# duwt/OrienMask

Measured on AMD Instinct MI355X. Metric: images/sec end-to-end (544^2, bs=32) forward+postprocess, higher is better.
Workload: dtype f32 (fp32 tensors and accumulation; products from hi/lo fp16 pairs of the fp32 operands, three fp16 MFMAs per product group)

## Files before the change

include/orienmask_hip.h:

```cpp
#ifndef ORIENMASK_HIP_H
#define ORIENMASK_HIP_H

#include <stddef.h>
#include <stdint.h>

#ifdef __cplusplus
extern "C" {
#endif

#define OM_VERSION 140

#define OM_OK 0
#define OM_EINVAL (-1)
#define OM_ESTATE (-2)
#define OM_ENOMEM (-3)
#define OM_EHIP (-4)

#define OM_MAX_SCALES 3
#define OM_MAX_ANCHORS 9

typedef struct om_model om_model;
typedef void* om_stream;

typedef struct om_layer_info {
// ... 89 lines not shown
                  void* out, int out_pix_stride, int out_f32, om_stream stream);
int om_conv2d_stem_f16(const float* in, int B, int H, int W, const float* w, const float* scale, const float* shift,
                       int cout, void* out, om_stream stream);
size_t om_conv2d_winograd24_scratch_bytes(int B, int H, int W, int cin);
int om_conv2d_winograd24(const float* in, int B, int H, int W, int cin, int in_pix_stride, const float* u,
                         const float* scale, const float* shift, int cout, int leaky, const float* res,
                         int res_pix_stride, float* out, int out_pix_stride, void* scratch, size_t scratch_bytes,
                         om_stream stream);
int om_conv2d_split(const float* in, int B, int H, int W, int cin, int in_pix_stride, const void* w_split,
                    const float* scale_split, const float* shift, int cout, int ksize, int stride, int leaky, const float* res,
                    int res_pix_stride, float* out, int out_pix_stride, int out_mode, int up, int tile_bm, int tile_bn,
                    int32_t* status_dev, om_stream stream);
int om_conv2d_split_k(const float* in, int B, int H, int W, int cin, int in_pix_stride, const void* w_split,
                      const float* scale_split, const float* shift, int cout, int ksize, int stride, int leaky, const float* res,
                      int res_pix_stride, float* out, int out_pix_stride, int out_mode, int up, int tile_bm, int tile_bn,
                      int max_parts, int32_t* status_dev, om_stream stream);
int om_conv2d_split_gather(int nseg, const float* const* seg_ptr, const int* seg_channels, const int* seg_pix_stride,
                           const int* seg_up, int B, int H, int W, const void* w_split, const float* scale_split, const float* shift,
                           int cout, int leaky, float* out, int out_pix_stride, int32_t* status_dev, om_stream stream);
int om_conv2d_winograd24_split(const float* in, int B, int H, int W, int cin, int in_pix_stride, const void* u_split,
                               const float* scale_split, const float* shift, int cout, int leaky, const float* res,
                               int res_pix_stride, float* out, int out_pix_stride, void* scratch, size_t scratch_bytes,
                               int32_t* status_dev, om_stream stream);
int om_conv2d_wino14_split(const float* in, int B, int H, int W, int cin, int in_pix_stride, const void* u14_split,
                           const float* scale_split, const float* shift, int cout, int leaky, const float* res,
                           int res_pix_stride, float* out, int out_pix_stride, int32_t* status_dev, om_stream stream);
size_t om_conv2d_wino14_wide_scratch_bytes(int B, int H, int W, int cin);
int om_conv2d_wino14_wide(const float* in, int B, int H, int W, int cin, int in_pix_stride, const void* u14_split,
                          const float* scale_split, const float* shift, int cout, int leaky, const float* res,
                          int res_pix_stride, float* out, int out_pix_stride, void* scratch, size_t scratch_bytes,
                          int32_t* status_dev, om_stream stream);
int om_set_wino14_wide(int on);
int om_get_wino14_wide(void);
int om_set_wino14_variant(int variant);
int om_get_wino14_variant(void);
int om_wino14_dual_built(void);
int om_set_stem_fusion(int which, int on);
int om_get_stem_fusion(int which);
int om_set_conv3x3_f16_variant(int mode);
int om_get_conv3x3_f16_variant(void);
int om_conv2d_stem(const float* in, int B, int H, int W, const float* w, const float* scale,
                   const float* shift, int cout, float* out, om_stream stream);
int om_conv2d_stem2_split(const float* in, int B, int H, int W, const float* w1, const float* scale1, const float* shift1,
                          const void* w2_split, const float* scale2_split, const float* shift2, int cout2, int leaky2, float* out,
                          int out_pix_stride, int32_t* status_dev, om_stream stream);
int om_conv2d_stem3_split(const float* in, int B, int H, int W, const float* w1, const float* scale1, const float* shift1,
                          const void* w2_split, const float* scale2_split, const float* shift2, int cout2, int leaky2, float* out,
                          int out_pix_stride, const void* w3_split, const float* scale3_split, const float* shift3, int cout3, int leaky3,
                          float* out3, int out3_pix_stride, int32_t* status_dev, om_stream stream);
int om_conv2d_stem2_f16(const float* in, int B, int H, int W, const float* w1, const float* scale1, const float* shift1,
                        const void* w2_f16, const float* scale2, const float* shift2, int cout2, int leaky2, void* out,
                        int out_pix_stride, om_stream stream);

int om_preprocess(const float* in_nhwc, int N, int h, int w, int resize_h, int resize_w, const float* mean3,
                  const float* std3, int pad_top, int pad_left, int out_h, int out_w, float pad_value, float* out_nchw,
                  om_stream stream);
int om_pad_nchw(const float* in, long long planes, int h, int w, int pad_top, int pad_left, int out_h, int out_w,
                float pad_value, float* out, om_stream stream);

size_t om_postprocess_workspace_bytes(const om_post_cfg* cfg, int B);
int om_postprocess(const om_post_cfg* cfg, const float* bbox32, const float* bbox16, const float* bbox8,
                   const float* oriens, int B, float* out_bbox, int64_t* out_cls, uint8_t* out_mask,
                   int32_t* out_count, int32_t* out_keep, void* workspace, size_t ws_bytes, om_stream stream);
int om_postprocess_detect(const om_post_cfg* cfg, const float* bbox32, const float* bbox16, const float* bbox8, int B,
                          float* out_bbox, int64_t* out_cls, int32_t* out_count, int32_t* out_keep, void* workspace, size_t ws_bytes,
                          om_stream stream);
// ... 119 lines not shown
```

orienmask_amd/csrc/conv_igemm_split.hip:

```cpp
#include <cstdlib>

#include "conv_f16_common.h"

namespace om {

#ifndef OM_SPLIT_WIDE
#define OM_SPLIT_WIDE 1
#endif

#if defined(OM_SPLIT_NO_XCD_PLACEMENT) && !defined(OM_MEASUREMENT_BUILD)
#error "OM_SPLIT_NO_XCD_PLACEMENT is a measurement switch: tools/build_variant.sh only"
#endif
#ifndef OM_SPLIT_TRACE
#define OM_SPLIT_TRACE 0
#endif
#if (OM_SPLIT_TRACE) && !defined(OM_MEASUREMENT_BUILD)
#error "measurement switches (wrong numerics / trace stores) are only for ab/ variants: build them with tools/build_variant.sh, which defines OM_MEASUREMENT_BUILD and never writes orienmask_amd/lib/"
#endif
#if OM_SPLIT_TRACE
static unsigned long long* g_split_trace = nullptr;
extern "C" void om_debug_split_trace(void* buf) { g_split_trace = static_cast<unsigned long long*>(buf); }
#define SPLIT_STAMP(x) asm volatile("s_memtime %0\n\ts_waitcnt lgkmcnt(0)" : "=s"(x)::"memory")
#endif

struct IgemmSParams {
    const _Float16* in;
    const _Float16* w;
    const float* scale;
    const float* shift;
    const float* res;
    float* out;
    int* ticket;
// ... 723 lines not shown
                            for (int g = 0; g < 4; ++g) {
                                const f32x4 v = __builtin_bit_cast(f32x4, __builtin_amdgcn_raw_buffer_load_b128(rs_part, qbase, ((a * TN + b) * 4 + g) * 256 * 16, 16));
#pragma unroll
                                for (int kk = 0; kk < 4; ++kk) acc[a][b][4 * g + kk] += v[kk];
                            }
                }
                asm volatile("s_waitcnt vmcnt(0)" ::: "memory");
            }
        }
#if OM_SPLIT_TRACE
        SPLIT_STAMP(ts2);
#endif

#if OM_SPLIT_TRACE
        SPLIT_STAMP(dts[4]);
#endif
        split_epilogue<BM, BN, WM, WN, FAST>(p, smem, acc, m0, n0, tid, wm, wn, fi, fk, sc, sh);
#if OM_SPLIT_TRACE
        if constexpr (KSPLIT) {
            asm volatile("s_waitcnt vmcnt(0)" ::: "memory");
            SPLIT_STAMP(dts[5]);
            deep_dump();
        }
        SPLIT_STAMP(ts3);
        if (p.trace && blockIdx.x < 16 && n_traced < 16 && tid == 0) {
            unsigned long long* t = p.trace + ((size_t)blockIdx.x * 16 + n_traced) * 8;
            t[0] = ts0; t[1] = ts1; t[2] = ts2; t[3] = ts3; t[4] = twait; t[5] = (unsigned long long)tile;
        }
        ++n_traced;
#endif
    }
}

template <int BM, int BN, int WM, int WN, bool WIDE = false, bool GATHER = false, int NBUF = 3, int WSTAGES = 0>
static int launch_tile_split(IgemmSParams p, int cout_pad, int blocks_per_cu, hipStream_t stream) {
    const int m_tiles = (p.M + BM - 1) / BM;
    p.n_tiles = cout_pad / BN;
    const long long total = (long long)m_tiles * p.n_tiles;
    OM_REQUIRE(total > 0 && total < (1ll << 31), OM_EINVAL, "conv split: %lld tiles out of range", total);
    p.total_tiles = (int)total;
    constexpr bool DEEP = WIDE ? WSTAGES > 2 : NBUF > 3;
    int parts = 1;
    if constexpr (DEEP) {
        if (p.ksplit > 1 && p.partial && total <= SK_SLOTS) {
            parts = p.ksplit;
            if (parts > 512 / (int)total) parts = 512 / (int)total;
            if (parts > p.ksteps / 16) parts = p.ksteps / 16;
            if (parts > 8) parts = 8;
            if (parts < 1) parts = 1;
        }
    }
    p.ksplit = parts;
    p.total_tickets = p.total_tiles * parts;
    p.m_tiles = m_tiles;
    const long long tickets = total * parts;
    long long grid = tickets < 256ll * blocks_per_cu ? tickets : 256ll * blocks_per_cu;
    if constexpr (DEEP) {
        OM_REQUIRE(tickets <= 512, OM_EINVAL, "conv split: %lld units in a deep-ring launch", tickets);
        grid = tickets;
    }
    const bool fast = p.out_mode == 0 && !p.res && p.vec_io && p.cout == cout_pad;
    if constexpr (WIDE) {
        constexpr int WNBUF = DEEP ? WSTAGES : 2;
        if (fast) hipLaunchKernelGGL((conv_igemm_split_wide_kernel<BM, BN, WM, WN, GATHER, true, WNBUF>), dim3((unsigned)grid), dim3(256), 0, stream, p);
        else hipLaunchKernelGGL((conv_igemm_split_wide_kernel<BM, BN, WM, WN, GATHER, false, WNBUF>), dim3((unsigned)grid), dim3(256), 0, stream, p);
    } else {
        if (fast) hipLaunchKernelGGL((conv_igemm_split_kernel<BM, BN, WM, WN, true, NBUF>), dim3((unsigned)grid), dim3(256), 0, stream, p);
        else hipLaunchKernelGGL((conv_igemm_split_kernel<BM, BN, WM, WN, false, NBUF>), dim3((unsigned)grid), dim3(256), 0, stream, p);
    }
    OM_CHECK_HIP(hipGetLastError());
    return OM_OK;
}

void conv_tile_for_split(int M, int cout_pad, int* bm, int* bn) {
    struct Cand { int bm, bn; double eff; };
    const Cand cands[] = {{128, 128, 1.00}, {256, 128, 0.91}, {128, 64, 0.82}, {64, 64, 0.69}, {128, 32, 0.57}};
    double best = 1e300;
    for (const Cand& c : cands) {
        if (cout_pad % c.bn) continue;
        const double cost = (double)((M + c.bm - 1) / c.bm) * (cout_pad / c.bn) * c.bm * c.bn / c.eff;
        if (cost < best) { best = cost; *bm = c.bm; *bn = c.bn; }
    }
#ifndef OM_SPLIT_NO_LATENCY_TILES
    const Cand small[] = {{128, 64, 0}, {64, 64, 0}};
    for (const Cand& c : small) {
        const long long tiles = (long long)((M + *bm - 1) / *bm) * (cout_pad / *bn);
        if (tiles > 128 || cout_pad % c.bn || c.bm * c.bn >= *bm * *bn) continue;
        *bm = c.bm; *bn = c.bn;
    }
#endif
}

int launch_conv_igemm_split(const ConvArgs& a, hipStream_t stream) {
    OM_REQUIRE((a.in || a.nseg > 0) && a.w && a.scale && a.shift && a.out, OM_EINVAL, "conv split: null pointer");
    OM_REQUIRE(a.cin % 16 == 0 && a.cin >= 16, OM_EINVAL, "conv split: cin=%d must be a multiple of 16", a.cin);
    OM_REQUIRE(a.ks == 1 || a.ks == 3, OM_EINVAL, "conv split: ksize=%d not supported", a.ks);
    OM_REQUIRE(a.stride == 1 || a.stride == 2, OM_EINVAL, "conv split: stride=%d not supported", a.stride);
    OM_REQUIRE((a.nseg > 0 || (a.in_pix_stride % 4 == 0 && (reinterpret_cast<uintptr_t>(a.in) & 15) == 0)) &&
                   (reinterpret_cast<uintptr_t>(a.w) & 15) == 0,
               OM_EINVAL, "conv split: input view / weights must be 16-byte aligned");
    OM_REQUIRE(a.cout_pad % 32 == 0 && a.cout <= a.cout_pad, OM_EINVAL, "conv split: cout_pad=%d", a.cout_pad);
    OM_REQUIRE((long long)a.B * a.H * a.W * a.in_pix_stride < (1ll << 40) && (long long)a.B * a.H * a.W < (1ll << 31) &&
// ... 17 lines not shown
    p.total_in_pixels = a.B * a.H * a.W;
    p.w_bytes = a.cout_pad * p.taps * a.cin * 4;
    p.vec_io = (a.out_mode != 2 && a.out_pix_stride % 4 == 0 && (reinterpret_cast<uintptr_t>(a.out) & 15) == 0 &&
                (!a.res || (a.res_pix_stride % 4 == 0 && (reinterpret_cast<uintptr_t>(a.res) & 15) == 0)))
                   ? 1 : 0;
    p.nseg = 0; p.nimg = a.B;
#if OM_SPLIT_TRACE
    p.trace = g_split_trace;
#endif
    for (int g = 0; g < 4; ++g) { p.seg_ptr[g] = p.in; p.seg_stride_h[g] = 0; p.seg_shift[g] = 0; p.seg_end[g] = 0x7FFFFFFF; }
    if (a.nseg > 0) {
        OM_REQUIRE(a.nseg <= 4 && a.ks == 1 && a.stride == 1 && a.cout_pad % 128 == 0, OM_EINVAL,
                   "conv split: a gathered input needs a 1x1 stride-1 layer with cout_pad %% 128 == 0 and at most 4 segments (nseg=%d ks=%d "
                   "stride=%d cout_pad=%d)", a.nseg, a.ks, a.stride, a.cout_pad);
        int end = 0;
        for (int g = 0; g < a.nseg; ++g) {
            const int up = a.seg_up[g];
            int sh = 0;
            while ((1 << sh) < up) ++sh;
            OM_REQUIRE(a.seg_ptr[g] && up >= 1 && (1 << sh) == up && a.H % up == 0 && a.W % up == 0 && a.seg_channels[g] > 0 &&
                           a.seg_channels[g] % 32 == 0 && a.seg_pix_stride[g] % 4 == 0 && a.seg_pix_stride[g] >= a.seg_channels[g] &&
                           (reinterpret_cast<uintptr_t>(a.seg_ptr[g]) & 15) == 0,
                       OM_EINVAL, "conv split: segment %d (channels=%d pix_stride=%d up=%d) of a gathered input", g, a.seg_channels[g],
                       a.seg_pix_stride[g], up);
            end += a.seg_channels[g] / 32;
            p.seg_ptr[g] = reinterpret_cast<const _Float16*>(a.seg_ptr[g]);
            p.seg_stride_h[g] = 2 * a.seg_pix_stride[g]; p.seg_shift[g] = sh; p.seg_end[g] = end;
        }
        OM_REQUIRE(end * 32 == a.cin, OM_EINVAL, "conv split: the segments hold %d channels, the layer reads %d", end * 32, a.cin);
        p.nseg = a.nseg;
        p.in = p.seg_ptr[0];
        return launch_tile_split<128, 128, 64, 64, true, true>(p, a.cout_pad, 2, stream);
    }
    int bm, bn;
    conv_tile_for_split(p.M, a.cout_pad, &bm, &bn);
    if (a.force_bm || a.force_bn) {
        const bool built = (a.force_bm == 256 && a.force_bn == 128) || (a.force_bm == 128 && (a.force_bn == 128 || a.force_bn == 64 || a.force_bn == 32)) ||
                           (a.force_bm == 64 && a.force_bn == 64);
        OM_REQUIRE(built && a.cout_pad % a.force_bn == 0, OM_EINVAL, "conv split: %d x %d is not a built tile shape for cout_pad=%d",
                   a.force_bm, a.force_bn, a.cout_pad);
        bm = a.force_bm; bn = a.force_bn;
    }
    if (bm == 256 && bn == 128) return launch_tile_split<256, 128, 128, 64>(p, a.cout_pad, 2, stream);
    if (bm == 128 && bn == 128 && a.cin % 32 == 0 && !a.force_bm && OM_SPLIT_WIDE) return launch_tile_split<128, 128, 64, 64, true>(p, a.cout_pad, 2, stream);
    if (bm == 128 && bn == 128) return launch_tile_split<128, 128, 64, 64>(p, a.cout_pad, 3, stream);
    const long long ntile = (long long)((p.M + bm - 1) / bm) * (a.cout_pad / bn);
    const bool deep = ntile <= 256 && (!a.force_bm || a.ksplit_max >= 1);
#ifndef OM_DEEP_WIDE
#define OM_DEEP_WIDE 1
#endif
    if (OM_DEEP_WIDE && deep && a.cin % 32 == 0) {
        if (bm == 128 && bn == 64) return launch_tile_split<128, 64, 64, 32, true, false, 3, 3>(p, a.cout_pad, 2, stream);
        if (bm == 64 && bn == 64) return launch_tile_split<64, 64, 32, 32, true, false, 3, 4>(p, a.cout_pad, 2, stream);
    }
    if (bm == 128 && bn == 64 && deep) return launch_tile_split<128, 64, 64, 32, false, false, 5>(p, a.cout_pad, 2, stream);
    if (bm == 64 && bn == 64 && deep) return launch_tile_split<64, 64, 32, 32, false, false, 8>(p, a.cout_pad, 2, stream);
#ifndef OM_SPLIT_WIDE_SMALLN
#define OM_SPLIT_WIDE_SMALLN 0
#endif
#if OM_SPLIT_WIDE_SMALLN
    if (bm == 128 && bn == 64 && a.cin % 32 == 0 && !a.force_bm) return launch_tile_split<128, 64, 64, 32, true>(p, a.cout_pad, OM_SPLIT_WIDE_SMALLN, stream);
    if (bm == 128 && bn == 32 && a.cin % 32 == 0 && !a.force_bm) return launch_tile_split<128, 32, 32, 32, true>(p, a.cout_pad, OM_SPLIT_WIDE_SMALLN + 1, stream);
#endif
    if (bm == 128 && bn == 64) return launch_tile_split<128, 64, 64, 32>(p, a.cout_pad, 4, stream);
    if (bm == 64 && bn == 64) return launch_tile_split<64, 64, 32, 32>(p, a.cout_pad, 4, stream);
    return launch_tile_split<128, 32, 32, 32>(p, a.cout_pad, 4, stream);
// ... 4 lines not shown
```

orienmask_amd/csrc/om_common.h:

```cpp
#pragma once
#include <hip/hip_runtime.h>
#include <cstdarg>
#include <cstdint>
#include <cstdio>

#include "../../include/orienmask_hip.h"

namespace om {

void set_error(const char* fmt, ...);

#define OM_CHECK_HIP(expr)                                                              \
    do {                                                                                \
        hipError_t _e = (expr);                                                         \
        if (_e != hipSuccess) {                                                         \
            om::set_error("%s failed: %s (%s:%d)", #expr, hipGetErrorString(_e), __FILE__, __LINE__); \
            return OM_EHIP;                                                             \
        }                                                                               \
    } while (0)

#define OM_REQUIRE(cond, code, ...)                                                     \
    do {                                                                                \
        if (!(cond)) {                                                                  \
            om::set_error(__VA_ARGS__);                                                 \
// ... 10 lines not shown
    const float* scale;
    const float* shift;
    const float* res;
    float* out;
    int* ticket = nullptr;
    float* sk_partial = nullptr;
    hipEvent_t mid_event = nullptr;
    int B, H, W, cin, in_pix_stride;
    int Ho, Wo, cout, cout_pad;
    int ks, stride;
    int leaky;
    int res_pix_stride;
    int out_pix_stride;
    int out_mode;
    int up;
    int split = 0;
    int* status = nullptr;
    int ksplit_max = 0;
    int force_bm = 0, force_bn = 0;
    int nseg = 0;
    const float* seg_ptr[4] = {nullptr, nullptr, nullptr, nullptr};
    int seg_channels[4] = {0, 0, 0, 0}, seg_pix_stride[4] = {0, 0, 0, 0}, seg_up[4] = {1, 1, 1, 1};
};

constexpr int SK_SLOTS = 1024;
constexpr int SK_FLAG_OFF = 16;
constexpr int SYNC_WORDS = SK_FLAG_OFF + SK_SLOTS;
constexpr int STATUS_WORDS = 16;
constexpr size_t SK_PARTIAL_BYTES = (size_t)512 * 32 * 256 * 16;

int launch_conv_igemm(const ConvArgs& a, hipStream_t stream);
int launch_conv_igemm_split(const ConvArgs& a, hipStream_t stream);
void conv_tile_for_split(int M, int cout_pad, int* bm, int* bn);

struct ConvArgsH {
    const void* in;
    const void* w;
    const float* scale;
    const float* shift;
    const void* res;
    void* out;
    int* ticket = nullptr;
    int B, H, W, cin, in_pix_stride;
    int Ho, Wo, cout, cout_pad;
    int ks, stride;
    int leaky;
    int res_pix_stride;
    int out_pix_stride;
    int out_mode;
    int up;
    int out_f32;
    int nseg = 0;
    const void* seg_ptr[4] = {nullptr, nullptr, nullptr, nullptr};
    int seg_channels[4] = {0, 0, 0, 0}, seg_pix_stride[4] = {0, 0, 0, 0}, seg_up[4] = {1, 1, 1, 1};
};
int launch_conv_igemm_f16(const ConvArgsH& a, hipStream_t stream);
int launch_conv3x3_f16(const ConvArgsH& a, hipStream_t stream);
bool conv3x3_f16_supported(const ConvArgsH& a);
void conv3x3_tile_for_f16(int M, int cout_pad, int W, int kc, int* bm, int* bn);
int conv3x3_f16_get_tall();
void conv3x3_f16_set_tall(int mode);
void conv_tile_for_f16(int M, int cout_pad, int cin, int* bm, int* bn);
inline size_t conv_f16_weight_halfs(int cout_pad, int ks, int cin) {
    return (size_t)cout_pad * ks * ks * cin;
}
int launch_conv_stem_f16(const float* in_nchw, int B, int H, int W, const float* w, const float* scale,
// ... 37 lines not shown
```

orienmask_amd/csrc/om_model.cpp:

```cpp
#include <algorithm>
#include <cstdlib>
#include <cstring>
#include <mutex>
#include <string>
#include <vector>

#include "om_common.h"

namespace om {

static thread_local char g_err[512] = "";

void set_error(const char* fmt, ...) {
    va_list ap;
    va_start(ap, fmt);
    vsnprintf(g_err, sizeof(g_err), fmt, ap);
    va_end(ap);
}

enum : int { BUF_INPUT = -1, BUF_BBOX32 = -2, BUF_BBOX16 = -3, BUF_BBOX8 = -4, BUF_ORIENS = -5 };
constexpr int HEAD_PIX_STRIDE = 256;

struct BufDef {
    int div;
// ... 889 lines not shown
    OM_REQUIRE(index >= 0 && index < (int)m->layers.size(), OM_EINVAL, "om_layer_tile: index %d", index);
    const om::LayerDef& L = m->layers[index];
    if (L.stem && m->stem2_fused((size_t)index)) { *bm = 128; *bn = 64; *algo = 9; return OM_OK; }
    if (L.stem) { *bm = 0; *bn = 0; *algo = 0; return OM_OK; }
    if (index == 1 && m->stem2_fused(0)) { *bm = 0; *bn = 0; *algo = 10; return OM_OK; }
    if (index == 2 && m->stem3_fused()) { *bm = 0; *bn = 0; *algo = 10; return OM_OK; }
    if (L.info.wino_off >= 0 && om::wino_enabled() && L.info.wino_planes == 24 && m->precision == 1 && m->direct_3x3_layer(L, B, H, W)) {
        om::conv_tile_for_split(B * (H / L.in_div) * (W / L.in_div), L.info.cout_pad, bm, bn);
        *algo = 7;
        return OM_OK;
    }
    if (L.info.wino_off >= 0 && om::wino_enabled() && L.info.wino_planes == 24 && m->precision == 1) {
        if (m->wide_3x3_layer(L, B, H, W)) { *algo = 12; *bm = 128; *bn = 128; return OM_OK; }
        *algo = 8; *bm = 128; *bn = 64;
        return OM_OK;
    }
    if (L.info.wino_off >= 0 && om::wino_enabled() && L.info.wino_planes == 24 && m->use_f24(B, H, W)) {
        *algo = 5; *bm = 64; *bn = 64;
        return OM_OK;
    }
    if (L.info.wino_off >= 0 && om::wino_enabled()) {
        const int Hl = H / L.in_div, Wl = W / L.in_div;
        *algo = om::wino_fused_for(L.info.cin) ? 3 : 2;
        *bm = 64;
        *bn = *algo == 3 ? (L.info.cout_pad % 128 == 0 ? 128 : 64)
                         : om::wino_bn((long long)B * ((Hl + 1) / 2) * ((Wl + 1) / 2), L.info.cout_pad);
        return OM_OK;
    }
    const int Ho = H / L.in_div / L.info.stride, Wo = W / L.in_div / L.info.stride;
    if (m->precision == 1 && L.info.wino_planes != 24) {
        om::conv_tile_for_split(B * Ho * Wo, L.info.cout_pad, bm, bn);
        *algo = 7;
        if (m->gather_active(false) && !L.gather.empty()) { *bm = 128; *bn = 128; *algo = 11; }
        return OM_OK;
    }
    om::conv_tile_for(B * Ho * Wo, L.info.cout_pad, bm, bn);
    *algo = 1;
    return OM_OK;
}

int om_profile_enable(om_model* m, int enable) {
    OM_REQUIRE(m, OM_EINVAL, "om_profile_enable: null model");
    m->profiling = enable != 0;
    m->prof_mask.clear();
    m->ev_used = 0;
    m->prof_forwards = 0;
    return OM_OK;
}

int om_profile_enable_layers(om_model* m, const unsigned char* layer_mask, int n_layers) {
    OM_REQUIRE(m && layer_mask, OM_EINVAL, "om_profile_enable_layers: null argument");
    OM_REQUIRE(n_layers == (int)m->layers.size(), OM_EINVAL, "om_profile_enable_layers: n_layers=%d, graph has %zu", n_layers,
               m->layers.size());
    m->profiling = true;
    m->prof_mask.assign(layer_mask, layer_mask + n_layers);
    m->ev_used = 0;
    m->prof_forwards = 0;
    return OM_OK;
}

int om_profile_read(om_model* m, float* layer_ms, float* layer_pre_ms, int n_layers, int* n_forwards) {
    OM_REQUIRE(m && layer_ms && layer_pre_ms && n_forwards, OM_EINVAL, "om_profile_read: null argument");
    OM_REQUIRE(n_layers == (int)m->layers.size(), OM_EINVAL, "om_profile_read: n_layers=%d, graph has %zu", n_layers,
               m->layers.size());
    size_t n_rec = 0;
    for (int i = 0; i < n_layers; ++i) n_rec += (m->prof_mask.empty() || m->prof_mask[i]) ? 1 : 0;
// ... 232 lines not shown

size_t om_conv2d_wino14_wide_scratch_bytes(int B, int H, int W, int cin) {
    if (B <= 0 || H <= 0 || W <= 0 || cin <= 0 || cin % 16) return 0;
    return om::align_up(om::wino14_wide_scratch_floats(B, H, W, cin) * sizeof(float), 256);
}

int om_conv2d_wino14_wide(const float* in, int B, int H, int W, int cin, int in_pix_stride, const void* u14_split,
                          const float* scale_split, const float* shift, int cout, int leaky, const float* res,
                          int res_pix_stride, float* out, int out_pix_stride, void* scratch, size_t scratch_bytes,
                          int32_t* status_dev, om_stream stream) {
    OM_REQUIRE(B > 0 && H > 0 && W > 0, OM_EINVAL, "om_conv2d_wino14_wide: bad shape");
    OM_REQUIRE(scratch && scratch_bytes >= om_conv2d_wino14_wide_scratch_bytes(B, H, W, cin), OM_ENOMEM,
               "om_conv2d_wino14_wide: scratch too small");
    om::ConvArgs a;
    a.in = in; a.w = static_cast<const float*>(u14_split); a.scale = scale_split; a.shift = shift; a.res = res; a.out = out;
    a.B = B; a.H = H; a.W = W; a.cin = cin; a.in_pix_stride = in_pix_stride;
    a.Ho = H; a.Wo = W; a.cout = cout; a.cout_pad = om::round_up(cout, 64);
    a.ks = 3; a.stride = 1; a.leaky = leaky; a.res_pix_stride = res_pix_stride;
    a.out_pix_stride = out_pix_stride; a.out_mode = 0; a.up = 1; a.split = 1; a.status = status_dev;
    static int* g_ticket = nullptr;
    if (!g_ticket) OM_CHECK_HIP(hipMalloc(reinterpret_cast<void**>(&g_ticket), om::SYNC_WORDS * sizeof(int)));
    if (int rc = om::launch_zero_words(g_ticket, om::SYNC_WORDS, static_cast<hipStream_t>(stream))) return rc;
    a.ticket = g_ticket;
    return om::launch_conv_wino14_wide(a, static_cast<float*>(scratch), static_cast<hipStream_t>(stream));
}

int om_set_wino14_wide(int on) {
    OM_REQUIRE(on == 0 || on == 1, OM_EINVAL, "om_set_wino14_wide: %d", on);
    g_wino14_wide = on;
    return OM_OK;
}
int om_get_wino14_wide(void) { return wino14_wide_on() ? 1 : 0; }

int om_wino14_dual_built(void) {
#ifdef OM_WITH_W14D
    return 1;
#else
    return 0;
#endif
}

int om_set_wino14_variant(int variant) {
    OM_REQUIRE(variant == 0 || variant == 1, OM_EINVAL, "om_set_wino14_variant: %d", variant);
    OM_REQUIRE(variant == 0 || om_wino14_dual_built(), OM_EINVAL,
               "om_set_wino14_variant: this library was built without the dual-role kernel (make W14D=1)");
    om::wino14_set_variant(variant);
    return OM_OK;
}

int om_conv2d_stem3_split(const float* in, int B, int H, int W, const float* w1, const float* scale1, const float* shift1,
                          const void* w2_split, const float* scale2_split, const float* shift2, int cout2, int leaky2, float* out,
                          int out_pix_stride, const void* w3_split, const float* scale3_split, const float* shift3, int cout3, int leaky3,
                          float* out3, int out3_pix_stride, int32_t* status_dev, om_stream stream) {
    om::Stem2Third third{w3_split, scale3_split, shift3, out3, cout3, leaky3, out3_pix_stride};
    return om::launch_conv_stem2_split(in, B, H, W, w1, scale1, shift1, w2_split, scale2_split, shift2, cout2, leaky2, out,
                                       out_pix_stride, status_dev, static_cast<hipStream_t>(stream), &third);
}

int om_conv2d_stem2_f16(const float* in, int B, int H, int W, const float* w1, const float* scale1, const float* shift1,
                        const void* w2_f16, const float* scale2, const float* shift2, int cout2, int leaky2, void* out, int out_pix_stride,
                        om_stream stream) {
    return om::launch_conv_stem2_f16(in, B, H, W, w1, scale1, shift1, w2_f16, scale2, shift2, cout2, leaky2, out, out_pix_stride,
                                     static_cast<hipStream_t>(stream));
}

int om_get_wino14_variant(void) { return om::wino14_variant(); }
// ... 34 lines not shown
```

orienmask_amd/lib.py:

```python
import ctypes
import os

_HERE = os.path.dirname(os.path.abspath(__file__))
LIB_PATH = os.path.join(_HERE, "lib", "liborienmask_hip.so")

OM_MAX_SCALES = 3
OM_MAX_ANCHORS = 9
OM_STATUS_SPLIT_RANGE = 1
OM_STATUS_SK_TIMEOUT = 2


class LayerInfo(ctypes.Structure):
    _fields_ = [("name", ctypes.c_char * 64),
                ("cin", ctypes.c_int32), ("cout", ctypes.c_int32), ("cout_pad", ctypes.c_int32),
                ("ksize", ctypes.c_int32), ("stride", ctypes.c_int32),
                ("has_bn", ctypes.c_int32), ("leaky", ctypes.c_int32), ("wino_planes", ctypes.c_int32),
                ("w_off", ctypes.c_int64), ("scale_off", ctypes.c_int64), ("shift_off", ctypes.c_int64),
                ("wino_off", ctypes.c_int64), ("wino_alt_off", ctypes.c_int64), ("w16_off", ctypes.c_int64),
                ("wsplit_off", ctypes.c_int64), ("wsplit_scale_off", ctypes.c_int64),
                ("wsplit_direct_off", ctypes.c_int64), ("wsplit_direct_scale_off", ctypes.c_int64)]


class PostCfg(ctypes.Structure):
    _fields_ = [("num_scales", ctypes.c_int32),
# ... 64 lines not shown
SIGNATURES = {
    "om_version": (_i, []),
    "om_last_error": (ctypes.c_char_p, []),
    "om_model_create": (_i, [ctypes.POINTER(_vp), _i, _i]),
    "om_model_create_variant": (_i, [ctypes.POINTER(_vp), _i, _i, _i]),
    "om_model_destroy": (None, [_vp]),
    "om_model_num_layers": (_i, [_vp]),
    "om_model_layer_info": (_i, [_vp, _i, ctypes.POINTER(LayerInfo)]),
    "om_model_weight_floats": (_sz, [_vp]),
    "om_model_load_weights": (_i, [_vp, _vp, _sz, _i]),
    "om_model_weight_split_words": (_sz, [_vp]),
    "om_model_load_weights_split": (_i, [_vp, _vp, _sz]),
    "om_model_set_precision": (_i, [_vp, _i]),
    "om_model_get_precision": (_i, [_vp]),
    "om_model_set_latency_cells": (_i, [_vp, ctypes.c_longlong]),
    "om_model_set_latency_ksplit": (_i, [_vp, _i]),
    "om_model_attach_postprocess": (_i, [_vp, ctypes.POINTER(PostCfg), _vp, _vp, _vp, _vp, _vp, _vp, ctypes.c_size_t]),
    "om_model_set_upsample_on_read": (_i, [_vp, _i]),
    "om_conv2d_split": (_i, [_vp, _i, _i, _i, _i, _i, _vp, _vp, _vp, _i, _i, _i, _i, _vp, _i, _vp, _i, _i, _i, _i, _i, _vp, _vp]),
    "om_conv2d_split_k": (_i, [_vp, _i, _i, _i, _i, _i, _vp, _vp, _vp, _i, _i, _i, _i, _vp, _i, _vp, _i, _i, _i, _i, _i, _i, _vp, _vp]),
    "om_conv2d_winograd24_split": (_i, [_vp, _i, _i, _i, _i, _i, _vp, _vp, _vp, _i, _i, _vp, _i, _vp, _i, _vp, _sz, _vp, _vp]),
    "om_set_wino14_variant": (_i, [_i]),
    "om_wino14_dual_built": (_i, []),
    "om_get_wino14_variant": (_i, []),
    "om_set_stem_fusion": (_i, [_i, _i]),
    "om_get_stem_fusion": (_i, [_i]),
    "om_get_conv3x3_f16_variant": (_i, []),
    "om_set_conv3x3_f16_variant": (_i, [_i]),
    "om_conv2d_wino14_split": (_i, [_vp, _i, _i, _i, _i, _i, _vp, _vp, _vp, _i, _i, _vp, _i, _vp, _i, _vp, _vp]),
    "om_conv2d_wino14_wide_scratch_bytes": (_sz, [_i, _i, _i, _i]),
    "om_conv2d_wino14_wide": (_i, [_vp, _i, _i, _i, _i, _i, _vp, _vp, _vp, _i, _i, _vp, _i, _vp, _i, _vp, _sz, _vp, _vp]),
    "om_set_wino14_wide": (_i, [_i]),
    "om_get_wino14_wide": (_i, []),
    "om_forward_workspace_bytes": (_sz, [_vp, _i, _i, _i]),
    "om_forward_status_offset": (_sz, [_vp, _i, _i, _i]),
    "om_forward": (_i, [_vp, _vp, _i, _i, _i, _vp, _vp, _vp, _vp, _vp, _sz, _vp]),
    "om_layer_tile": (_i, [_vp, _i, _i, _i, _i, ctypes.POINTER(ctypes.c_int), ctypes.POINTER(ctypes.c_int),
                           ctypes.POINTER(ctypes.c_int)]),
    "om_model_weight_halfs": (_sz, [_vp]),
    "om_model_load_weights_f16": (_i, [_vp, _vp, _sz]),
    "om_forward_f16_workspace_bytes": (_sz, [_vp, _i, _i, _i]),
    "om_forward_f16": (_i, [_vp, _vp, _i, _i, _i, _vp, _vp, _vp, _vp, _vp, _sz, _vp]),
    "om_layer_tile_f16": (_i, [_vp, _i, _i, _i, _i, ctypes.POINTER(ctypes.c_int), ctypes.POINTER(ctypes.c_int),
                               ctypes.POINTER(ctypes.c_int)]),
    "om_conv2d_f16": (_i, [_vp, _i, _i, _i, _i, _i, _vp, _vp, _vp, _i, _i, _i, _i, _vp, _i, _vp, _i, _i, _vp]),
    "om_conv2d_stem_f16": (_i, [_vp, _i, _i, _i, _vp, _vp, _vp, _i, _vp, _vp]),
    "om_conv2d_winograd_scratch_bytes": (_sz, [_i, _i, _i, _i]),
    "om_conv2d_winograd": (_i, [_vp, _i, _i, _i, _i, _i, _vp, _vp, _vp, _i, _i, _vp, _i, _vp, _i, _vp, _sz, _vp]),
    "om_layer_output_view": (_i, [_vp, _i, _i, _i, _i, _i, ctypes.POINTER(ctypes.c_size_t), ctypes.POINTER(ctypes.c_int),
                                  ctypes.POINTER(ctypes.c_int), ctypes.POINTER(ctypes.c_int)]),
    "om_model_keep_activations": (_i, [_vp, _i]),
    "om_conv2d_winograd24_scratch_bytes": (_sz, [_i, _i, _i, _i]),
    "om_conv2d_winograd24": (_i, [_vp, _i, _i, _i, _i, _i, _vp, _vp, _vp, _i, _i, _vp, _i, _vp, _i, _vp, _sz, _vp]),
    "om_profile_enable": (_i, [_vp, _i]),
    "om_profile_enable_layers": (_i, [_vp, ctypes.c_char_p, _i]),
    "om_profile_read": (_i, [_vp, ctypes.POINTER(ctypes.c_float), ctypes.POINTER(ctypes.c_float), _i,
                             ctypes.POINTER(ctypes.c_int)]),
    "om_conv2d": (_i, [_vp, _i, _i, _i, _i, _i, _vp, _vp, _vp, _i, _i, _i, _i, _vp, _i, _vp, _i, _vp]),
    "om_conv2d_mode": (_i, [_vp, _i, _i, _i, _i, _i, _vp, _vp, _vp, _i, _i, _i, _i, _vp, _i, _vp, _i, _i, _i, _vp]),
    "om_conv2d_stem": (_i, [_vp, _i, _i, _i, _vp, _vp, _vp, _i, _vp, _vp]),
    "om_conv2d_stem2_split": (_i, [_vp, _i, _i, _i, _vp, _vp, _vp, _vp, _vp, _vp, _i, _i, _vp, _i, _vp, _vp]),
    "om_conv2d_stem3_split": (_i, [_vp, _i, _i, _i, _vp, _vp, _vp, _vp, _vp, _vp, _i, _i, _vp, _i, _vp, _vp, _vp, _i, _i, _vp, _i, _vp, _vp]),
    "om_conv2d_stem2_f16": (_i, [_vp, _i, _i, _i, _vp, _vp, _vp, _vp, _vp, _vp, _i, _i, _vp, _i, _vp]),
    "om_conv2d_split_gather": (_i, [_i, ctypes.POINTER(_vp), ctypes.POINTER(_i), ctypes.POINTER(_i), ctypes.POINTER(_i), _i, _i, _i,
                                    _vp, _vp, _vp, _i, _i, _vp, _i, _vp, _vp]),
    "om_preprocess": (_i, [_vp, _i, _i, _i, _i, _i, ctypes.POINTER(ctypes.c_float), ctypes.POINTER(ctypes.c_float),
# ... 80 lines not shown
```

Baseline: 2181.

## Add persistent streaming 256x128 split-fp16 kernel for large 1x1 convs

Adds a persistent, one-block-per-CU kernel for 1x1 stride-1 convs with cin=256 and many tiles. Each block takes tiles from an atomic ticket counter and keeps a 6-deep LDS ring of async buffer loads running across tile boundaries, so the next tile's prologue loads overlap the current tile's MFMAs and epilogue. It uses larger 256x128 tiles with 8 waves. It is on by default, can be turned off through an env var or a setter, and adds complex vmcnt accounting that could hide subtle hazards.

Measured after the change: 2186, median of 4. No clear change (+0.2%).

```diff
diff --git a/include/orienmask_hip.h b/include/orienmask_hip.h
--- a/include/orienmask_hip.h
+++ b/include/orienmask_hip.h
@@ -145,6 +145,8 @@
                           int32_t* status_dev, om_stream stream);
 int om_set_wino14_wide(int on);
 int om_get_wino14_wide(void);
+int om_set_split_stream(int on);
+int om_get_split_stream(void);
 int om_set_wino14_variant(int variant);
 int om_get_wino14_variant(void);
 int om_wino14_dual_built(void);
diff --git a/orienmask_amd/csrc/conv_igemm_split.hip b/orienmask_amd/csrc/conv_igemm_split.hip
--- a/orienmask_amd/csrc/conv_igemm_split.hip
+++ b/orienmask_amd/csrc/conv_igemm_split.hip
@@ -1,3 +1,4 @@
+#include <atomic>
 #include <cstdlib>
 
 #include "conv_f16_common.h"
@@ -787,6 +788,191 @@
     }
 }
 
+constexpr int SS_BM = 256, SS_BN = 128, SS_NBUF = 6;
+constexpr int SS_STAGE = (SS_BM + SS_BN) * 4;
+constexpr int SS_CAREA = 32 * SS_BN / 4;
+static_assert((SS_NBUF * SS_STAGE + SS_CAREA) * 16 <= 160 * 1024, "LDS budget");
+
+template <int KSTEPS>
+__global__ __launch_bounds__(512, 1) void conv_igemm_split_stream_kernel(const IgemmSParams p) {
+    constexpr int BM = SS_BM, BN = SS_BN, WM = 64, WN = 64, TM = 2, TN = 2, NBUF = SS_NBUF, STAGE = SS_STAGE;
+    constexpr int NP = 3;
+    constexpr int E = 16;
+    constexpr int W_STEADY = (NBUF - 2) * NP;
+    static_assert(KSTEPS >= 2 * NBUF, "the ticket drawn at k-step 0 is read at k-step KSTEPS - NBUF - 1, NBUF - 1 waits later");
+    __shared__ f32x4 smem[NBUF * STAGE + SS_CAREA];
+    f32x4* const sC = smem + NBUF * STAGE;
+    int* const s_ticket = reinterpret_cast<int*>(sC + 128);
+
+    const int tid = threadIdx.x;
+    const int lane = tid & 63;
+    const int wave = tid >> 6;
+    const int wave_u = __builtin_amdgcn_readfirstlane(wave);
+    const int wm = wave >> 1, wn = wave & 1;
+    const int lrow = tid >> 2, lcol = tid & 3;
+    const int scol = lcol ^ ((lrow >> 2) & 3);
+    const int fi = lane & 31, fk = lane >> 5;
+    const int fsw = (fi >> 2) & 3;
+
+    int ld_tile = 0, ld_in_bytes = 0, ld_w_bytes = 0;
+    unsigned ld_in_lo = 0, ld_in_hi = 0, ld_w_soff = 0;
+    const int ld_rowA0 = (lrow * p.in_pix_stride_h + scol * 8) * 2;
+    const int ld_rowA1 = ((lrow + 128) * p.in_pix_stride_h + scol * 8) * 2;
+    const int ld_rowB = (lrow * p.cin_h + scol * 8) * 2;
+    auto set_loader = [&](int t) {
+        ld_tile = t;
+        const bool live = t < p.total_tiles;
+        const int tt = live ? t : 0;
+        const int m0 = (tt / p.n_tiles) * BM, n0 = (tt % p.n_tiles) * BN;
+        const unsigned long long base = reinterpret_cast<unsigned long long>(p.in + (size_t)m0 * p.in_pix_stride_h);
+        ld_in_lo = __builtin_amdgcn_readfirstlane((unsigned)base);
+        ld_in_hi = __builtin_amdgcn_readfirstlane((unsigned)(base >> 32));
+        const long long left = (long long)(p.M - m0) * p.in_pix_stride_h * 2;
+        ld_in_bytes = __builtin_amdgcn_readfirstlane(live ? (left < 0x7FFFFFFFll ? (int)left : 0x7FFFFFFF) : 0);
+        ld_w_bytes = __builtin_amdgcn_readfirstlane(live ? p.w_bytes : 0);
+        ld_w_soff = __builtin_amdgcn_readfirstlane((unsigned)(n0 * p.cin_h * 2));
+    };
+    auto issue_stage = [&](int k, int buf) {
+        f32x4* dst = smem + buf * STAGE + wave_u * 64;
+        const _Float16* in = reinterpret_cast<const _Float16*>(((unsigned long long)ld_in_hi << 32) | ld_in_lo);
+        const auto rs_in = __builtin_amdgcn_make_buffer_rsrc(const_cast<_Float16*>(in), 0, ld_in_bytes, 0x00020000);
+        const auto rs_w = __builtin_amdgcn_make_buffer_rsrc(const_cast<_Float16*>(p.w), 0, ld_w_bytes, 0x00020000);
+        __builtin_amdgcn_raw_ptr_buffer_load_lds(rs_in, (lds_ptr_t)(dst), 16, ld_rowA0 + k * 64, 0, 0, 0);
+        __builtin_amdgcn_raw_ptr_buffer_load_lds(rs_in, (lds_ptr_t)(dst + 512), 16, ld_rowA1 + k * 64, 0, 0, 0);
+        __builtin_amdgcn_raw_ptr_buffer_load_lds(rs_w, (lds_ptr_t)(dst + BM * 4), 16, ld_rowB + k * 64, ld_w_soff, 0, 0);
+    };
+
+    if (tid == 0) *s_ticket = atomicAdd(p.ticket, 1);
+    asm volatile("s_waitcnt lgkmcnt(0)" ::: "memory");
+    __builtin_amdgcn_s_barrier();
+    set_loader(__builtin_amdgcn_readfirstlane(*s_ticket));
+    if (ld_tile >= p.total_tiles) return;
+    int buf = 0;
+#pragma unroll
+    for (int st = 0; st < NBUF; ++st) issue_stage(st, st);
+
+    const f32x4* fragA = smem + (wm * WM + fi) * 4;
+    const f32x4* fragB = smem + BM * 4 + (wn * WN + fi) * 4;
+    f32x4 xa0[TM], xa1[TM], nbh[TN], nbl[TN];
+    f16x8 ah[TM], al[TM], bh[TN], bl[TN];
+    auto read_raw = [&](int b) {
+        const int c0 = fk ^ fsw, c1 = (2 + fk) ^ fsw;
+        const int bo = b * STAGE;
+#pragma unroll
+        for (int a = 0; a < TM; ++a) { xa0[a] = fragA[bo + a * 32 * 4 + c0]; xa1[a] = fragA[bo + a * 32 * 4 + c1]; }
+#pragma unroll
+        for (int b2 = 0; b2 < TN; ++b2) { nbh[b2] = fragB[bo + b2 * 32 * 4 + c0]; nbl[b2] = fragB[bo + b2 * 32 * 4 + c1]; }
+    };
+    auto convert = [&]() {
+#pragma unroll
+        for (int a = 0; a < TM; ++a) split8(xa0[a], xa1[a], ah[a], al[a]);
+#pragma unroll
+        for (int b = 0; b < TN; ++b) { bh[b] = __builtin_bit_cast(f16x8, nbh[b]); bl[b] = __builtin_bit_cast(f16x8, nbl[b]); }
+    };
+
+    for (bool first = true;; first = false) {
+        const int tile = ld_tile;
+        if (tile >= p.total_tiles) break;
+        const int m0 = (tile / p.n_tiles) * BM, n0 = (tile % p.n_tiles) * BN;
+
+        if (first) asm volatile("s_waitcnt vmcnt(%0)" ::"i"((NBUF - 1) * NP) : "memory");
+        else asm volatile("s_waitcnt vmcnt(%0)" ::"i"((NBUF - 1) * NP + E) : "memory");
+        __builtin_amdgcn_s_barrier();
+        read_raw(buf);
+        convert();
+
+        f32x16 acc[TM][TN];
+#pragma unroll
+        for (int a = 0; a < TM; ++a)
+#pragma unroll
+            for (int b = 0; b < TN; ++b)
+#pragma unroll
+                for (int r = 0; r < 16; ++r) acc[a][b][r] = 0.f;
+
+        int next_ticket = 0;
+#pragma unroll
+        for (int s = 0; s < KSTEPS; ++s) {
+            const int buf1 = buf == NBUF - 1 ? 0 : buf + 1;
+            if (s < KSTEPS - 1) {
+                if (s + 1 <= NBUF - 1 && !first) asm volatile("s_waitcnt vmcnt(%0) lgkmcnt(0)" ::"i"(W_STEADY + E) : "memory");
+                else asm volatile("s_waitcnt vmcnt(%0) lgkmcnt(0)" ::"i"(W_STEADY) : "memory");
+            } else {
+                asm volatile("s_waitcnt lgkmcnt(0)" ::: "memory");
+            }
+            __builtin_amdgcn_s_barrier();
+            if (s == KSTEPS - NBUF) set_loader(__builtin_amdgcn_readfirstlane(*s_ticket));
+            if (s < KSTEPS - 1) read_raw(buf1);
+            if (s == 0 && tid == 0) next_ticket = (int)atomicInc(reinterpret_cast<unsigned*>(p.ticket), 0x7FFFFFFFu);
+            issue_stage(s + NBUF < KSTEPS ? s + NBUF : s + NBUF - KSTEPS, buf);
+            if (s == 0 && wave_u == 0) {
+                const auto rs_sc = __builtin_amdgcn_make_buffer_rsrc(const_cast<float*>(p.scale), 0, (p.n_tiles * BN) * 4, 0x00020000);
+                const auto rs_sh = __builtin_amdgcn_make_buffer_rsrc(const_cast<float*>(p.shift), 0, (p.n_tiles * BN) * 4, 0x00020000);
+                __builtin_amdgcn_raw_ptr_buffer_load_lds(rs_sc, (lds_ptr_t)(sC), 16, (n0 + lane * 4) * 4, 0, 0, 0);
+                __builtin_amdgcn_raw_ptr_buffer_load_lds(rs_sh, (lds_ptr_t)(sC + 64), 16, (n0 + lane * 4) * 4, 0, 0, 0);
+            }
+            if (s == KSTEPS - NBUF - 1 && tid == 0) *s_ticket = next_ticket;
+#pragma unroll
+            for (int a = 0; a < TM; ++a)
+#pragma unroll
+                for (int b = 0; b < TN; ++b) {
+                    acc[a][b] = __builtin_amdgcn_mfma_f32_32x32x16_f16(bh[b], al[a], acc[a][b], 0, 0, 0);
+                    acc[a][b] = __builtin_amdgcn_mfma_f32_32x32x16_f16(bl[b], ah[a], acc[a][b], 0, 0, 0);
+                    acc[a][b] = __builtin_amdgcn_mfma_f32_32x32x16_f16(bh[b], ah[a], acc[a][b], 0, 0, 0);
+                }
+            if (s < KSTEPS - 1) convert();
+            buf = buf1;
+        }
+
+        const int n8 = tid & 15, r = tid >> 4;
+        const int n = n0 + n8 * 8;
+        float sc[8], sh[8];
+        {
+            const float* scf = reinterpret_cast<const float*>(sC);
+#pragma unroll
+            for (int k = 0; k < 8; ++k) { sc[k] = scf[n8 * 8 + k]; sh[k] = scf[256 + n8 * 8 + k]; }
+        }
+        asm volatile("s_waitcnt lgkmcnt(0)" ::: "memory");
+        __builtin_amdgcn_s_barrier();
+        float* const out_base = p.out + (size_t)m0 * p.out_pix_stride;
+        const size_t out_left = (size_t)(p.M - m0) * p.out_pix_stride * 4;
+        const auto rs_out = __builtin_amdgcn_make_buffer_rsrc(out_base, 0, out_left < 0x7FFFFFFFull ? (int)out_left : 0x7FFFFFFF, 0x00020000);
+        float nonfinite = 0.f;
+#pragma unroll
+        for (int pass = 0; pass < BM / 32; ++pass) {
+            const int pw = pass >> 1, pa = pass & 1;
+            if (wm == pw) {
+#pragma unroll
+                for (int b = 0; b < TN; ++b)
+#pragma unroll
+                    for (int g = 0; g < 4; ++g) {
+                        const int n4 = (wn * WN + b * 32) / 4 + 2 * g + fk;
+                        f32x4 v = {acc[pa][b][4 * g], acc[pa][b][4 * g + 1], acc[pa][b][4 * g + 2], acc[pa][b][4 * g + 3]};
+                        sC[fi * (BN / 4) + (n4 ^ (fi & 7))] = v;
+                    }
+            }
+            asm volatile("s_waitcnt lgkmcnt(0)" ::: "memory");
+            __builtin_amdgcn_s_barrier();
+            const f32x4 v0 = sC[r * (BN / 4) + ((2 * n8) ^ (r & 7))];
+            const f32x4 v1 = sC[r * (BN / 4) + ((2 * n8 + 1) ^ (r & 7))];
+            float v[8] = {v0[0], v0[1], v0[2], v0[3], v1[0], v1[1], v1[2], v1[3]};
+#pragma unroll
+            for (int k = 0; k < 8; ++k) {
+                const float t = fmaf(v[k], sc[k], sh[k]);
+                v[k] = p.leaky ? (t > 0.f ? t : t * 0.1f) : t;
+                nonfinite = fmaf(t, 0.f, nonfinite);
+            }
+            const int off = ((pass * 32 + r) * p.out_pix_stride + n) * 4;
+            typedef __attribute__((__vector_size__(4 * sizeof(unsigned)))) unsigned u32x4;
+            __builtin_amdgcn_raw_buffer_store_b128(__builtin_bit_cast(u32x4, f32x4{v[0], v[1], v[2], v[3]}), rs_out, off, 0, 0);
+            __builtin_amdgcn_raw_buffer_store_b128(__builtin_bit_cast(u32x4, f32x4{v[4], v[5], v[6], v[7]}), rs_out, off + 16, 0, 0);
+            asm volatile("s_waitcnt lgkmcnt(0)" ::: "memory");
+            __builtin_amdgcn_s_barrier();
+        }
+        if (p.status && nonfinite != nonfinite) atomicOr(p.status, OM_STATUS_SPLIT_RANGE);
+    }
+    asm volatile("s_waitcnt vmcnt(0)" ::: "memory");
+}
+
 template <int BM, int BN, int WM, int WN, bool WIDE = false, bool GATHER = false, int NBUF = 3, int WSTAGES = 0>
 static int launch_tile_split(IgemmSParams p, int cout_pad, int blocks_per_cu, hipStream_t stream) {
     const int m_tiles = (p.M + BM - 1) / BM;
@@ -823,6 +1009,51 @@
         if (fast) hipLaunchKernelGGL((conv_igemm_split_kernel<BM, BN, WM, WN, true, NBUF>), dim3((unsigned)grid), dim3(256), 0, stream, p);
         else hipLaunchKernelGGL((conv_igemm_split_kernel<BM, BN, WM, WN, false, NBUF>), dim3((unsigned)grid), dim3(256), 0, stream, p);
     }
+    OM_CHECK_HIP(hipGetLastError());
+    return OM_OK;
+}
+
+static std::atomic<int> g_split_stream{-1};
+void set_split_stream(int on) { g_split_stream.store(on ? 1 : 0); }
+bool split_stream_on() {
+    int v = g_split_stream.load();
+    if (v < 0) {
+        const char* e = std::getenv("OM_NO_SPLIT_STREAM");
+        v = (e && e[0] == '1') ? 0 : 1;
+        int expected = -1;
+        g_split_stream.compare_exchange_strong(expected, v);
+        v = g_split_stream.load();
+    }
+    return v != 0;
+}
+
+static int device_cu_count() {
+    static std::atomic<int> cached[64];
+    int dev = 0;
+    if (hipGetDevice(&dev) != hipSuccess || dev < 0 || dev >= 64) return 256;
+    int n = cached[dev].load();
+    if (n <= 0) {
+        if (hipDeviceGetAttribute(&n, hipDeviceAttributeMultiprocessorCount, dev) != hipSuccess || n <= 0) n = 256;
+        cached[dev].store(n);
+    }
+    return n;
+}
+
+bool split_stream_selected(int M, int cin, int ks, int stride, int cout, int cout_pad, bool plain_out) {
+    if (!split_stream_on() || ks != 1 || stride != 1 || !plain_out || cin != 16 * 16 || cout != cout_pad || cout_pad % SS_BN) return false;
+    const long long tiles = (long long)((M + SS_BM - 1) / SS_BM) * (cout_pad / SS_BN);
+    return tiles >= 4ll * device_cu_count();
+}
+
+static int launch_split_stream(IgemmSParams p, int cout_pad, hipStream_t stream) {
+    const int m_tiles = (p.M + SS_BM - 1) / SS_BM;
+    p.n_tiles = cout_pad / SS_BN;
+    p.total_tiles = m_tiles * p.n_tiles;
+    p.m_tiles = m_tiles;
+    p.ksplit = 1; p.total_tickets = p.total_tiles;
+    OM_REQUIRE(p.ksteps == 16 && p.taps == 1, OM_EINVAL, "conv split stream: %d k-steps, %d taps", p.ksteps, p.taps);
+    const int grid = p.total_tiles < device_cu_count() ? p.total_tiles : device_cu_count();
+    hipLaunchKernelGGL((conv_igemm_split_stream_kernel<16>), dim3((unsigned)grid), dim3(512), 0, stream, p);
     OM_CHECK_HIP(hipGetLastError());
     return OM_OK;
 }
@@ -906,6 +1137,9 @@
         p.in = p.seg_ptr[0];
         return launch_tile_split<128, 128, 64, 64, true, true>(p, a.cout_pad, 2, stream);
     }
+    if (!a.force_bm && !a.force_bn && p.vec_io &&
+        split_stream_selected(p.M, a.cin, a.ks, a.stride, a.cout, a.cout_pad, a.out_mode == 0 && !a.res))
+        return launch_split_stream(p, a.cout_pad, stream);
     int bm, bn;
     conv_tile_for_split(p.M, a.cout_pad, &bm, &bn);
     if (a.force_bm || a.force_bn) {
diff --git a/orienmask_amd/csrc/om_common.h b/orienmask_amd/csrc/om_common.h
--- a/orienmask_amd/csrc/om_common.h
+++ b/orienmask_amd/csrc/om_common.h
@@ -66,6 +66,9 @@
 int launch_conv_igemm(const ConvArgs& a, hipStream_t stream);
 int launch_conv_igemm_split(const ConvArgs& a, hipStream_t stream);
 void conv_tile_for_split(int M, int cout_pad, int* bm, int* bn);
+bool split_stream_selected(int M, int cin, int ks, int stride, int cout, int cout_pad, bool plain_out);
+void set_split_stream(int on);
+bool split_stream_on();
 
 struct ConvArgsH {
     const void* in;
diff --git a/orienmask_amd/csrc/om_model.cpp b/orienmask_amd/csrc/om_model.cpp
--- a/orienmask_amd/csrc/om_model.cpp
+++ b/orienmask_amd/csrc/om_model.cpp
@@ -945,6 +945,8 @@
         om::conv_tile_for_split(B * Ho * Wo, L.info.cout_pad, bm, bn);
         *algo = 7;
         if (m->gather_active(false) && !L.gather.empty()) { *bm = 128; *bn = 128; *algo = 11; }
+        else if (om::split_stream_selected(B * Ho * Wo, L.info.cin, L.info.ksize, L.info.stride, L.info.cout, L.info.cout_pad,
+                                           !L.has_res && L.out_mode == 0)) { *bm = 256; *bn = 128; }
         return OM_OK;
     }
     om::conv_tile_for(B * Ho * Wo, L.info.cout_pad, bm, bn);
@@ -1243,6 +1245,13 @@
 }
 int om_get_wino14_wide(void) { return wino14_wide_on() ? 1 : 0; }
 
+int om_set_split_stream(int on) {
+    OM_REQUIRE(on == 0 || on == 1, OM_EINVAL, "om_set_split_stream: %d", on);
+    om::set_split_stream(on);
+    return OM_OK;
+}
+int om_get_split_stream(void) { return om::split_stream_on() ? 1 : 0; }
+
 int om_wino14_dual_built(void) {
 #ifdef OM_WITH_W14D
     return 1;
diff --git a/orienmask_amd/lib.py b/orienmask_amd/lib.py
--- a/orienmask_amd/lib.py
+++ b/orienmask_amd/lib.py
@@ -120,6 +120,8 @@
     "om_conv2d_wino14_wide": (_i, [_vp, _i, _i, _i, _i, _i, _vp, _vp, _vp, _i, _i, _vp, _i, _vp, _i, _vp, _sz, _vp, _vp]),
     "om_set_wino14_wide": (_i, [_i]),
     "om_get_wino14_wide": (_i, []),
+    "om_set_split_stream": (_i, [_i]),
+    "om_get_split_stream": (_i, []),
     "om_forward_workspace_bytes": (_sz, [_vp, _i, _i, _i]),
     "om_forward_status_offset": (_sz, [_vp, _i, _i, _i]),
     "om_forward": (_i, [_vp, _vp, _i, _i, _i, _vp, _vp, _vp, _vp, _vp, _sz, _vp]),
```
